# sakehl/SKA-SDP-Accelerate-gridding

Measured on AMD Instinct MI355X. Metric: Mvis/s gridded (w-proj, 4096^2 grid), higher is better.
Workload: dtype f64

## Files before the change

ska-sdp-accelerate-gridding_amd/csrc/tile_sorted.hip:

```cpp
#include "tile_common.h"

namespace gridhip {

__device__ __forceinline__ double readlane_f64(double x, int l)
{
    return __hiloint2double(__builtin_amdgcn_readlane(__double2hiint(x), l),
                            __builtin_amdgcn_readlane(__double2loint(x), l));
}

constexpr int SORTED_IM_OFF = 65528;

__device__ const int cut15[3][16] = {{0, 106, 211, 317, 422, 500, 578, 655, 733, 781, 829, 877, 926, 958, 991, 1024},
                                     {0, 108, 221, 329, 434, 513, 596, 677, 754, 800, 852, 898, 943, 969, 998, 1024},
                                     {0, 100, 202, 303, 401, 480, 562, 641, 718, 769, 824, 875, 925, 957, 992, 1024}};

struct SortedItem {
    int32_t valid, tile, grp, staged;
};

template <int S, bool DEGRID, int ABL = 0, bool AW = false, bool BT = false>
__global__ void __launch_bounds__(1024, 4) tile_grid_sorted_kernel(Geom g, const RecWord *__restrict__ recs,
                                                                const int32_t *__restrict__ bin_start,
                                                                const int32_t *__restrict__ work_start,
                                                                const double2 *__restrict__ gcf,
                                                                double2 *__restrict__ vis,
                                                                double *__restrict__ grid, int nkeys, int batch,
                                                                int32_t *__restrict__ scalars,
                                                                double2 *__restrict__ sorted_vals,
                                                                uint2 *__restrict__ sorted_mo)
{
    extern __shared__ double lds[];
    constexpr int S2 = S * S;
    constexpr int TAIL0 = S2 - ((S2 + 63) / 64 - 1) * 64;
    constexpr int EXTRA = DEGRID ? 0 : (TAIL0 > 32 && TAIL0 <= 34) ? TAIL0 - 32 : (S2 > 256 && TAIL0 <= 2) ? TAIL0 : 0;
    constexpr int S2E = S2 - EXTRA;
    constexpr int NSTEP_ALL = (S2E + 63) / 64;
    constexpr int TAIL = S2E - (NSTEP_ALL - 1) * 64;
    constexpr int MAXST = DEGRID ? 4 : 5;
    constexpr int FP = (NSTEP_ALL + MAXST - 1) / MAXST;
    constexpr int KST = (NSTEP_ALL + FP - 1) / FP;
    constexpr int REM = NSTEP_ALL % FP;
    constexpr int PBASE = NSTEP_ALL / FP;
    constexpr int NSTEP = KST;
    constexpr int LASTS = (REM == 0 ? KST : KST - 1) - 1;
    constexpr bool PAIR = !DEGRID && TAIL == 32;
    const int tid = threadIdx.x, nthr = blockDim.x;
    const int lane = tid & 63, wave = __builtin_amdgcn_readfirstlane(tid >> 6), nw = nthr >> 6;
    const int plane = g.lrows * g.ldw;
    const int IMO = BT ? g.imoff / 8 : SORTED_IM_OFF / 8;
    double *lre = lds, *lim = lds + IMO;
    int32_t *hist = reinterpret_cast<int32_t *>(lim + plane);
    const int hist_words = (nkeys + 1 + 3) & ~3;
    SortedItem *desc = reinterpret_cast<SortedItem *>(hist + hist_words);
    double2 *svals_wg = sorted_vals + (size_t)blockIdx.x * 2 * batch;
    uint2 *smo_wg = sorted_mo + (size_t)blockIdx.x * 2 * batch;
    int32_t *sorig_wg = reinterpret_cast<int32_t *>(sorted_vals) + (size_t)blockIdx.x * 2 * batch;

    constexpr bool STAGE_VALS = !DEGRID && AW;
    constexpr bool STAGE_ORIG = DEGRID && AW;
    const bool solo = nw == 1;
    const bool is_sorter = wave == nw - 1;
    if (is_sorter && !solo && !(g.dbg & 512)) __builtin_amdgcn_s_setprio(3);
    const bool is_walker = solo || !is_sorter;
    const int nwalk = solo ? 1 : nw - 1;
    const int ncell = g.lrows * g.lcols;

    if (blockIdx.x == 0 && tid == 0) {
        long long *st = reinterpret_cast<long long *>(scalars + 20);
        st[0] = (long long)__builtin_amdgcn_s_memtime();
        st[1] = (long long)__builtin_amdgcn_s_memrealtime();
    }
    long long prof[7] = {0, 0, 0, 0, 0, 0, 0}, pt = 0;
#define GH_STAMP(i_)                        \
    if ((ABL & 16) && lane == 0) {          \
        const long long now_ = clock64();   \
        prof[i_] += now_ - pt;              \
        pt = now_;                          \
    }
    if ((ABL & 16) && lane == 0) pt = clock64();

    int32_t *queue = scalars + 4;
    int turn = 0;
    int items_left = ((int)blockIdx.x >= g.npersist) ? g.budget : 0x7fffffff;
    auto prepare = [&](int slot) {
        WorkItem w;
        int grp = 0;
        bool have = false;
        if (items_left <= 0) turn = g.ngroups;
        --items_left;
        while (turn < g.ngroups) {
            grp = (blockIdx.x + turn) % g.ngroups;
            int item = 0;
            if (lane == 0) item = atomicAdd(&queue[grp], 1);
            item = __builtin_amdgcn_readfirstlane(item);
            if (find_work_at(g, bin_start, work_start, grp, item, &w)) {
                have = true;
                break;
            }
            ++turn;
        }
        if (!have) {
            if (lane == 0) desc[slot].valid = 0;
            return;
        }
        GH_STAMP(0)
        const int first_plane = (grp * g.W + g.ngroups - 1) / g.ngroups;
        const int first_slice = first_plane * g.Q * g.Q * g.P;
        double2 *svals = svals_wg + (size_t)slot * batch;
        uint2 *smo = smo_wg + (size_t)slot * batch;
        int32_t *sorig = sorig_wg + (size_t)slot * batch;
        const int b_lo = w.v_lo;
        const int cnt = min(batch, w.v_hi - b_lo);
        for (int i = lane; i <= nkeys; i += 64) hist[i] = 0;
        __builtin_amdgcn_fence(__ATOMIC_ACQ_REL, "wavefront");
        __builtin_amdgcn_wave_barrier();
        for (int r0 = lane; r0 < cnt; r0 += 8 * 64) {
            int key[8];
#pragma unroll
            for (int q = 0; q < 8; ++q) {
                bool off;
                key[q] = load_rec(recs, b_lo + min(r0 + q * 64, cnt - 1), g, &off).kslice - first_slice;
                if (AW) key[q] = (int)((unsigned)key[q] % (unsigned)nkeys);
                if (off) key[q] = -1;
            }
#pragma unroll
            for (int q = 0; q < 8; ++q)
                if (r0 + q * 64 < cnt && (unsigned)key[q] < (unsigned)nkeys) atomicAdd(&hist[key[q]], 1);
        }
        __builtin_amdgcn_fence(__ATOMIC_ACQ_REL, "wavefront");
        __builtin_amdgcn_wave_barrier();
        GH_STAMP(1)
        {
            const int per = (nkeys + 63) / 64;
            const int lo = min(lane * per, nkeys), hi = min(lo + per, nkeys);
            int sum = 0;
            for (int i = lo; i < hi; ++i) sum += hist[i];
            int incl = sum;
#pragma unroll
            for (int off = 1; off < 64; off <<= 1) {
                const int t = __shfl_up(incl, off, 64);
                if (lane >= off) incl += t;
            }
            int base = incl - sum;
            for (int i = lo; i < hi; ++i) {
                const int c = hist[i];
                hist[i] = base;
                base += c;
            }
        }
        __builtin_amdgcn_fence(__ATOMIC_ACQ_REL, "wavefront");
        __builtin_amdgcn_wave_barrier();
        GH_STAMP(2)
        int bad = 0;
        for (int r0 = lane; r0 < cnt; r0 += 8 * 64) {
            VisRec rec[8];
            double2 val[8];
            bool off[8];
#pragma unroll
            for (int q = 0; q < 8; ++q) rec[q] = load_rec(recs, b_lo + min(r0 + q * 64, cnt - 1), g, &off[q]);
            if (STAGE_VALS) {
#pragma unroll
                for (int q = 0; q < 8; ++q) val[q] = (ABL & 8) ? make_double2(1.0, (double)q) : load_nt(vis + rec[q].orig);
            }
#pragma unroll
            for (int q = 0; q < 8; ++q) {
                if (r0 + q * 64 >= cnt) break;
                int key = rec[q].kslice - first_slice;
                if (AW) key = (int)((unsigned)key % (unsigned)nkeys);
                if (off[q] || (unsigned)key >= (unsigned)nkeys) {
                    ++bad;
                    continue;
                }
                const int pos = atomicAdd(&hist[key], 1);
                if ((unsigned)pos < (unsigned)batch) {
                    smo[pos] = make_uint2(((uint32_t)key << 16) | (uint32_t)((rec[q].lxy >> 16) * g.ldw + (rec[q].lxy & 0xffff)),
                                          (uint32_t)(AW ? rec[q].kslice : rec[q].orig));
                    if (STAGE_VALS) svals[pos] = val[q];
                    if (STAGE_ORIG) sorig[pos] = rec[q].orig;
                } else
                    ++bad;
            }
        }
        if (bad) atomicAdd(&scalars[2], bad);
        __builtin_amdgcn_fence(__ATOMIC_ACQ_REL, "wavefront");
        __builtin_amdgcn_wave_barrier();
        if (lane == 0) {
            SortedItem d;
            d.valid = 1;
            d.tile = w.tile;
            d.grp = grp;
            d.staged = hist[nkeys - 1];
            desc[slot] = d;
        }
        GH_STAMP(3)
    };

    int loff[NSTEP];
    const bool tail_ok = lane < TAIL || TAIL == 64;
#pragma unroll
    for (int s = 0; s < NSTEP; ++s) {
        int t = s * 64 + lane;
        if (FP == 1 && s == NSTEP - 1 && !tail_ok) t = PAIR ? s * 64 + lane - 32 : 0;
        loff[s] = (t / S) * g.ldw + (t % S);
    }
    const int ttail = tail_ok ? LASTS * 64 + lane : PAIR ? LASTS * 64 + lane - 32 : 0;
    const int lrow = lane / S, lcol = lane - lrow * S;

    auto walk = [&](int slot, int staged, int first_slice) {
        const double2 *svals = svals_wg + (size_t)slot * batch;
        const uint2 *smo = smo_wg + (size_t)slot * batch;
        const int32_t *sorig = sorig_wg + (size_t)slot * batch;
        int seg_lo, seg_hi;
        if (nwalk == 15 && !DEGRID && !(g.dbg & 256)) {
            seg_lo = (int)(((int64_t)staged * cut15[g.dense][wave]) >> 10);
            seg_hi = (int)(((int64_t)staged * cut15[g.dense][wave + 1]) >> 10);
        } else {
            seg_lo = (int)(((int64_t)staged * wave) / nwalk);
            seg_hi = (int)(((int64_t)staged * (wave + 1)) / nwalk);
        }
        if (seg_lo >= seg_hi) return;
        auto load_list = [&](int b0, uint2 &mo, double2 &v, int32_t &o) {
            const int idx = max(min(b0 + lane, seg_hi - 1), seg_lo);
            mo = smo[idx];
            if (STAGE_VALS) v = svals[idx];
            if (STAGE_ORIG) o = sorig[idx];
        };
        auto load_value = [&](const uint2 &mo, double2 &v) {
            if (!DEGRID && !STAGE_VALS) v = (ABL & 8) ? make_double2(1.0, 2.0) : load_nt(vis + mo.y);
        };
        auto part_step0 = [&](int part) { return FP == 1 ? 0 : part * PBASE + min(part, REM); };
        auto part_nst = [&](int part) { return (FP == 1 || REM == 0 || part < REM) ? KST : KST - 1; };
        auto issue = [&](double2(&k)[NSTEP], int key, int len, int part) {
            key = min(max(key, 0), (AW ? g.nslices : nkeys) - 1);
            asm volatile("" : "+s"(key));
            const double2 *kp = gcf + (size_t)(first_slice + key) * S2 + 64 * part_step0(part);
            if (ABL & 4) {
#pragma unroll
                for (int s = 0; s < NSTEP; ++s) k[s] = make_double2((double)key, (double)(lane + s));
                return;
            }
            const int lofs = len > 0 ? lane : 0, lt = len > 0 ? ttail : 0;
            if (FP == 1) {
#pragma unroll
                for (int s = 0; s < NSTEP - 1; ++s) k[s] = kp[s * 64 + lofs];
                k[NSTEP - 1] = kp[lt];
            } else {
                const bool lastp = part == FP - 1, shortp = part_nst(part) < KST;
#pragma unroll
                for (int s = 0; s < NSTEP; ++s) {
                    int idx = s * 64 + lofs;
                    if (s == LASTS && lastp) idx = lt;
                    if (s == KST - 1 && shortp) idx = 0;
                    k[s] = kp[idx];
                }
            }
        };
        uint2 moN, moNN;
        double2 vN = make_double2(0.0, 0.0), vNN = make_double2(0.0, 0.0);
        int32_t oN = 0, oNN = 0;
        load_list(seg_lo, moN, vN, oN);
        load_list(seg_lo + 64, moNN, vNN, oNN);
        load_value(moN, vN);
        for (int b0 = seg_lo; b0 < seg_hi; b0 += 64) {
            const uint2 mo = moN;
            const double2 vB = vN;
            const int32_t oB = oN;
            moN = moNN;
            vN = vNN;
            oN = oNN;
            load_value(moN, vN);
            load_list(b0 + 128, moNN, vNN, oNN);
            const int bcnt = min(64, seg_hi - b0);
            const uint32_t mykey = AW ? mo.y : mo.x >> 16;
            const uint32_t prevkey = (uint32_t)__shfl_up((int)mykey, 1, 64);
            unsigned long long bits = __ballot(lane < bcnt && (lane == 0 || mykey != prevkey));
            double2 kx[EXTRA > 0 ? EXTRA : 1];
            if (EXTRA > 0) {
                const double2 *kp = gcf + (size_t)(first_slice + min((int)mykey, (AW ? g.nslices : nkeys) - 1)) * S2 + (S2 - EXTRA);
#pragma unroll
                for (int e = 0; e < EXTRA; ++e) kx[e] = (ABL & 4) ? make_double2(1.0, 2.0) : kp[e];
            }
            int lastKey = 0;
            int curKey = 0, curStart = 0, curLen = 0, curPart = FP - 1;
            auto advance = [&](int &key, int &start, int &len, int &part) {
                if (FP > 1 && curLen > 0 && curPart < FP - 1) {
                    ++curPart;
                    key = curKey;
                    start = curStart;
                    len = curLen;
                    part = curPart;
                    return;
                }
                if (bits == 0) {
                    key = lastKey;
                    start = 0;
                    len = 0;
                    if (FP > 1) part = FP - 1;
                    curLen = 0;
                    return;
                }
                start = (int)__builtin_ctzll(bits);
                bits &= bits - 1;
                len = (bits ? (int)__builtin_ctzll(bits) : bcnt) - start;
                key = lastKey = AW ? __builtin_amdgcn_readlane((int)mo.y, start)
                                   : (int)((uint32_t)__builtin_amdgcn_readlane((int)mo.x, start) >> 16);
                if (FP > 1) {
                    part = 0;
                    curKey = key;
                    curStart = start;
                    curLen = len;
                    curPart = 0;
                }
            };
            auto process = [&](const double2(&k)[NSTEP], int start, int len, int part) {
                int lo[NSTEP];
                const bool lastp = FP == 1 || part == FP - 1;
                const bool shortp = FP > 1 && part_nst(part) < KST;
                if (FP == 1) {
#pragma unroll
                    for (int s = 0; s < NSTEP; ++s) lo[s] = loff[s];
                } else {
                    const int st0 = part_step0(part);
#pragma unroll
                    for (int s = 0; s < NSTEP; ++s) {
                        const int tl = 64 * (st0 + s);
                        const int A = tl / S, B = tl - A * S;
                        int lr = lrow, lc = lcol;
                        if (PAIR && s == LASTS && lastp && lane >= 32) {
                            lr = (lane - 32) / S;
                            lc = (lane - 32) - lr * S;
                        }
                        const int carry = (B + lc >= S) ? g.ldw - S : 0;
                        lo[s] = (A + lr) * g.ldw + B + lc + carry;
                    }
                }
                if (!DEGRID) {
                    int i = 0;
                    if (PAIR && lastp) {
                        for (; i + 1 < len; i += 2) {
                            const int j0 = start + i, j1 = j0 + 1;
                            const int lb0 = (int)((uint32_t)__builtin_amdgcn_readlane((int)mo.x, j0) & 0xffff);
                            const int lb1 = (int)((uint32_t)__builtin_amdgcn_readlane((int)mo.x, j1) & 0xffff);
                            const double vx0 = readlane_f64(vB.x, j0), vy0 = readlane_f64(vB.y, j0);
                            const double vx1 = readlane_f64(vB.x, j1), vy1 = readlane_f64(vB.y, j1);
#pragma unroll
                            for (int s = 0; s < LASTS; ++s) {
                                double *cell = lre + (lb0 + lo[s]);
                                if (ABL & 1) continue;
                                __hip_atomic_fetch_add(cell, vx0 * k[s].x - vy0 * k[s].y, __ATOMIC_RELAXED,
                                                       __HIP_MEMORY_SCOPE_WORKGROUP);
                                __hip_atomic_fetch_add(cell + IMO, vx0 * k[s].y + vy0 * k[s].x,
                                                       __ATOMIC_RELAXED, __HIP_MEMORY_SCOPE_WORKGROUP);
                            }
#pragma unroll
                            for (int s = 0; s < LASTS; ++s) {
                                double *cell = lre + (lb1 + lo[s]);
                                if (ABL & 1) continue;
                                __hip_atomic_fetch_add(cell, vx1 * k[s].x - vy1 * k[s].y, __ATOMIC_RELAXED,
                                                       __HIP_MEMORY_SCOPE_WORKGROUP);
                                __hip_atomic_fetch_add(cell + IMO, vx1 * k[s].y + vy1 * k[s].x,
                                                       __ATOMIC_RELAXED, __HIP_MEMORY_SCOPE_WORKGROUP);
                            }
                            const double2 kl = k[LASTS];
                            double re, im;
                            int a;
                            if (lane < 32) {
                                re = vx0 * kl.x - vy0 * kl.y;
                                im = vx0 * kl.y + vy0 * kl.x;
                                a = lb0 + lo[LASTS];
                                asm volatile("" : "+v"(a));
                            } else {
                                re = vx1 * kl.x - vy1 * kl.y;
                                im = vx1 * kl.y + vy1 * kl.x;
                                a = lb1 + lo[LASTS];
                                asm volatile("" : "+v"(a));
                            }
                            if (!(ABL & 1)) {
                                __hip_atomic_fetch_add(lre + a, re, __ATOMIC_RELAXED, __HIP_MEMORY_SCOPE_WORKGROUP);
                                __hip_atomic_fetch_add(lre + a + IMO, im, __ATOMIC_RELAXED,
                                                       __HIP_MEMORY_SCOPE_WORKGROUP);
                            }
                        }
                    }
                    for (; i < len; ++i) {
                        const int j = start + i;
                        const uint32_t m = (uint32_t)__builtin_amdgcn_readlane((int)mo.x, j);
                        const int lbase = (int)(m & 0xffff);
                        const double vx = readlane_f64(vB.x, j), vy = readlane_f64(vB.y, j);
#pragma unroll
                        for (int s = 0; s < NSTEP; ++s) {
                            if (FP > 1 && s == KST - 1 && shortp) continue;
                            const double re = vx * k[s].x - vy * k[s].y;
                            const double im = vx * k[s].y + vy * k[s].x;
                            double *cell = lre + (lbase + lo[s]);
                            if (ABL & 1) {
                                if (re == 1.2345e300 || im == 1.2345e300) *cell = re;
                                continue;
                            }
                            if (TAIL == 64 || s != LASTS || !lastp || tail_ok) {
                                __hip_atomic_fetch_add(cell, re, __ATOMIC_RELAXED, __HIP_MEMORY_SCOPE_WORKGROUP);
                                __hip_atomic_fetch_add(cell + IMO, im, __ATOMIC_RELAXED,
                                                       __HIP_MEMORY_SCOPE_WORKGROUP);
                            }
                        }
                    }
                } else {
                    const double2 kz = tail_ok ? k[LASTS] : make_double2(0.0, 0.0);
                    for (int i = 0; i < len; i += 4) {
                        double sr[4], si[4];
                        int32_t oo[4];
#pragma unroll
                        for (int q = 0; q < 4; ++q) {
                            sr[q] = 0.0;
                            si[q] = 0.0;
                            oo[q] = 0;
                            if (i + q < len) {
                                const int j = start + i + q;
                                const uint32_t m = (uint32_t)__builtin_amdgcn_readlane((int)mo.x, j);
                                const int lbase = (int)(m & 0xffff);
                                oo[q] = __builtin_amdgcn_readlane(STAGE_ORIG ? (int)oB : (int)mo.y, j);
                                double gr[NSTEP], gi[NSTEP];
#pragma unroll
                                for (int s = 0; s < NSTEP; ++s) {
                                    const bool nostep = FP > 1 && s == KST - 1 && shortp;
                                    const bool idle = TAIL != 64 && s == LASTS && lastp && !tail_ok;
                                    const double *cell = lre + (lbase + ((idle || nostep) ? lo[0] : lo[s]));
                                    gr[s] = cell[0];
                                    gi[s] = cell[IMO];
                                }
#pragma unroll
                                for (int s = 0; s < NSTEP; ++s) {
                                    double2 kk = (TAIL != 64 && s == LASTS && lastp) ? kz : k[s];
                                    if (FP > 1 && s == KST - 1 && shortp) kk = make_double2(0.0, 0.0);
                                    sr[q] = fma(kk.x, gr[s], sr[q]);
                                    sr[q] = fma(-kk.y, gi[s], sr[q]);
                                    si[q] = fma(kk.x, gi[s], si[q]);
                                    si[q] = fma(kk.y, gr[s], si[q]);
                                }
                            }
                        }
                        const double rr = wave_sum4_rows(sr[0], sr[1], sr[2], sr[3]);
                        const double ri = wave_sum4_rows(si[0], si[1], si[2], si[3]);
                        const int row = lane >> 4;
                        if ((lane & 15) == 15 && i + row < len) {
                            const int32_t o = row == 0 ? oo[0] : row == 1 ? oo[1] : row == 2 ? oo[2] : oo[3];
                            if (g.P == 1 && FP == 1)
                                __builtin_nontemporal_store(dvec2_t{rr, ri}, reinterpret_cast<dvec2_t *>(vis + o));
                            else {
                                double *dst = reinterpret_cast<double *>(vis + o);
                                unsafeAtomicAdd(dst, rr);
                                unsafeAtomicAdd(dst + 1, ri);
                            }
                        }
                    }
                }
            };

            constexpr int NSETS = 3;
            double2 kS[NSETS][NSTEP];
            int keyS[NSETS], startS[NSETS], lenS[NSETS], partS[NSETS] = {0, 0, 0};
            static_assert(NSETS == 3, "initialiser of partS");
#pragma unroll
            for (int r = 0; r < NSETS - 1; ++r) {
                advance(keyS[r], startS[r], lenS[r], partS[r]);
                issue(kS[r], keyS[r], lenS[r], partS[r]);
            }
            int done = 0;
            for (;;) {
#pragma unroll
                for (int r = 0; r < NSETS; ++r) {
                    const int nx = (r + NSETS - 1) % NSETS;
                    advance(keyS[nx], startS[nx], lenS[nx], partS[nx]);
                    issue(kS[nx], keyS[nx], lenS[nx], partS[nx]);
                    asm volatile("" ::: "memory");
                    __builtin_amdgcn_sched_barrier(0);
                    process(kS[r], startS[r], lenS[r], partS[r]);
                    __builtin_amdgcn_sched_barrier(0);
                    if (FP == 1 || partS[r] == FP - 1) done += lenS[r];
                }
                if (done >= bcnt) break;
            }
            if (done > bcnt) {
#pragma unroll
                for (int r = 0; r < NSETS - 1; ++r) asm volatile("" ::"v"(kS[r][0].x), "v"(kS[r][NSTEP - 1].y));
            }
            if (EXTRA > 0 && !(ABL & 1) && lane < bcnt) {
                const int lb = (int)(mo.x & 0xffff);
#pragma unroll
                for (int e = 0; e < EXTRA; ++e) {
                    const int t = S2 - EXTRA + e;
                    double *cell = lre + (lb + (t / S) * g.ldw + (t % S));
                    __hip_atomic_fetch_add(cell, vB.x * kx[e].x - vB.y * kx[e].y, __ATOMIC_RELAXED,
                                           __HIP_MEMORY_SCOPE_WORKGROUP);
                    __hip_atomic_fetch_add(cell + IMO, vB.x * kx[e].y + vB.y * kx[e].x, __ATOMIC_RELAXED,
                                           __HIP_MEMORY_SCOPE_WORKGROUP);
                }
            }
        }
    };

    const int fl_r0 = (tid >> 1) / g.lcols, fl_c0 = (tid >> 1) - fl_r0 * g.lcols;
    const int fl_dr = (nthr >> 1) / g.lcols, fl_dc = (nthr >> 1) - fl_dr * g.lcols;

    if (is_sorter) prepare(0);
    if (!DEGRID) {
        for (int i = tid; i < plane; i += nthr) {
            lre[i] = 0.0;
            lim[i] = 0.0;
        }
    }
    __syncthreads();
    for (int cur = 0;; cur ^= 1) {
        const SortedItem d = desc[cur];
        if (!d.valid) break;
        const int first_plane = (d.grp * g.W + g.ngroups - 1) / g.ngroups;
        const int first_slice = first_plane * g.Q * g.Q * g.P;
        const int tx = d.tile % g.ntx, ty = d.tile / g.ntx;
        const int64_t ox = (int64_t)tx * g.Tx - g.offx, oy = (int64_t)ty * g.Ty - g.offy;
        if (DEGRID) {
            const double2 *gsrc = reinterpret_cast<const double2 *>(grid);
            for (int c = tid; c < ncell; c += nthr) {
                const int r_ = c / g.lcols, c_ = c - r_ * g.lcols;
                const int64_t gx = ox + c_, gy = oy + r_;
                double2 v = make_double2(0.0, 0.0);
                if (gx >= 0 && gy >= 0 && gx < g.Wd && gy < g.H) v = gsrc[gy * g.Wd + gx];
                lre[r_ * g.ldw + c_] = v.x;
                lim[r_ * g.ldw + c_] = v.y;
            }
            __syncthreads();
        }
        const long long walk_t0 = (ABL & 16) ? clock64() : 0;
        if (is_sorter && !solo) prepare(cur ^ 1);
        if (is_walker) {
            if ((ABL & 16) && wave == 0 && lane == 0) pt = clock64();
            walk(cur, d.staged, first_slice);
            if ((ABL & 16) && wave == 0) GH_STAMP(4)
        }
        if (solo) prepare(cur ^ 1);
        if ((ABL & 16) && lane == 0)
            atomicAdd(reinterpret_cast<unsigned long long *>(scalars + 32) + 8 + wave, (unsigned long long)(clock64() - walk_t0));
        __syncthreads();
        if ((ABL & 16) && wave == 0) GH_STAMP(5)
        if (DEGRID) continue;

        {
            const int comp = tid & 1;
            int r_ = fl_r0, c_ = fl_c0;
            for (int e = tid; e < 2 * ncell; e += nthr) {
                const int64_t gx = ox + c_, gy = oy + r_;
                double *cell = (comp ? lim : lre) + r_ * g.ldw + c_;
                c_ += fl_dc;
                r_ += fl_dr;
                if (c_ >= g.lcols) {
                    c_ -= g.lcols;
                    ++r_;
                }
                const double val = *cell;
                if (val == 0.0) continue;
                *cell = 0.0;
                if ((ABL & 2) || gx < 0 || gy < 0 || gx >= g.Wd || gy >= g.H) continue;
                unsafeAtomicAdd(grid + 2 * (gy * g.Wd + gx) + comp, val);
            }
        }
        __syncthreads();
        if ((ABL & 16) && wave == 0) GH_STAMP(6)
    }
    if (blockIdx.x == 0 && tid == 0) {
        long long *st = reinterpret_cast<long long *>(scalars + 20);
        st[2] = (long long)__builtin_amdgcn_s_memtime();
        st[3] = (long long)__builtin_amdgcn_s_memrealtime();
    }
    if ((ABL & 16) && lane == 0 && (wave == 0 || (is_sorter && !solo))) {
        unsigned long long *out = reinterpret_cast<unsigned long long *>(scalars + 32);
        for (int i = 0; i < 7; ++i)
            if (prof[i]) atomicAdd(&out[i], (unsigned long long)prof[i]);
    }
#undef GH_STAMP
}

bool sorted_plan(const gridhip_ctx *ctx, const Geom &g, int block, int *nkeys, int *batch, size_t *lds_bytes)
{
    if (g.gh != g.gw || g.gh < 5 || g.gh > (g.per_vis ? 16 : 32)) return false;
    const int planes = (g.W + g.ngroups - 1) / g.ngroups + 1;
    const int64_t keys = g.per_vis ? 4096 : (int64_t)planes * g.Q * g.Q * g.P;
    if (keys >= 65536) return false;
    const size_t plane = (size_t)g.lrows * g.ldw * 8;
    if (plane > (size_t)(g.imoff > 0 ? g.imoff : SORTED_IM_OFF)) return false;
    const size_t tile = (size_t)(g.imoff > 0 ? g.imoff : SORTED_IM_OFF) + plane;
    const size_t hist = (size_t)((keys + 1 + 3) & ~3) * 4;
    if (tile + hist + 128 > (size_t)ctx->max_lds) return false;
    (void)block;
    int c = ctx->opt.chunk ? (int)ctx->opt.chunk : 16384;
    c = c < 64 ? 64 : c > 16384 ? 16384 : c;
    *nkeys = (int)keys;
    *batch = c;
    *lds_bytes = tile + hist + 128;
    return true;
}

int launch_tile_grid_sorted(gridhip_ctx *ctx, const Geom &g_in, int block, size_t lds_bytes, int nkeys, int batch,
                            int64_t n, const double *gcf, const double *vis, double *grid, bool degrid)
{
    Geom g = g_in;
    Tables t = tables_of(ctx, g);
    const RecWord *recs = (const RecWord *)ctx->recs.ptr;
    if (g.chunk > batch) return fail(ctx, GRIDHIP_EINVAL, "sorted kernel: chunk %d exceeds its work-item capacity %d", g.chunk, batch);
    if (g.per_vis && g.imoff > 0) return fail(ctx, GRIDHIP_EUNSUPPORTED, "no big-tile form of the aw tile kernel");
    int per_cu = (int)((size_t)ctx->max_lds / lds_bytes);
    per_cu = per_cu < 1 ? 1 : per_cu > 4 ? 4 : per_cu;
    if (per_cu * block > 2048) per_cu = 2048 / block > 0 ? 2048 / block : 1;
    int cus = ctx->num_cu - (int)ctx->opt.reserve_cus;
    if (cus < g.ngroups) cus = g.ngroups;
    int nblk = cus * per_cu;
    nblk = ctx->opt.reserve_cus ? (nblk / g.ngroups) * g.ngroups : ((nblk + g.ngroups - 1) / g.ngroups) * g.ngroups;
    const int most = work_blocks(g, n);
    if (nblk > most) nblk = most > g.ngroups ? (most / g.ngroups) * g.ngroups : g.ngroups;
    g.npersist = nblk;
    g.budget = 0;
    if (ctx->opt.yield_cus > 0 && !ctx->opt.reserve_cus) {
        int k = (((int)ctx->opt.yield_cus + 31) / 32) * 32 * per_cu;
        k = (k / g.ngroups) * g.ngroups;
        if (k > 0 && nblk - k >= g.ngroups) {
            g.npersist = nblk - k;
            g.budget = 8;
            int extra = most - g.npersist;
            extra = extra > 2048 ? 2048 : extra;
            extra = (extra / g.ngroups) * g.ngroups;
            nblk = g.npersist + (extra > k ? extra : k);
        }
    }
    const dim3 gr(nblk), bl(block);
    const size_t nlist = (size_t)nblk * 2 * batch, nvals = g.per_vis ? nlist : 0;
    GH_CHECK(ws_reserve(ctx, ctx->sorted, nvals * 16 + nlist * 8));
    double2 *svals = (double2 *)ctx->sorted.ptr;
    uint2 *smo = (uint2 *)(svals + nvals);
    launch_clear(ctx, t.scalars + 4, 16, (g.dbg & 16) ? t.scalars + 32 : nullptr, (g.dbg & 16) ? 64 : 0);
#define GH_LAUNCH_(S_, D_, B_)                                                                                   \
    do {                                                                                                         \
        GH_CHECK(raise_lds(ctx, tile_grid_sorted_kernel<S_, D_, 0, false, B_>));                                 \
        hipLaunchKernelGGL((tile_grid_sorted_kernel<S_, D_, 0, false, B_>), gr, bl, lds_bytes, ctx->stream, g, recs, \
                           t.bin_start, t.work_start, (const double2 *)gcf, (double2 *)vis, grid, nkeys, batch, \
                           t.scalars, svals, smo);                                                               \
    } while (0)
#define GH_LAUNCH(S_, D_)                \
    do {                                 \
        if (g.imoff > 0)                 \
            GH_LAUNCH_(S_, D_, true);    \
        else                             \
            GH_LAUNCH_(S_, D_, false);   \
    } while (0)
#define GH_LAUNCH_AW_(S_, D_)                                                                                    \
    do {                                                                                                         \
        GH_CHECK(raise_lds(ctx, tile_grid_sorted_kernel<S_, D_, 0, true>));                                      \
        hipLaunchKernelGGL((tile_grid_sorted_kernel<S_, D_, 0, true>), gr, bl, lds_bytes, ctx->stream, g, recs,  \
                           t.bin_start, t.work_start, (const double2 *)gcf, (double2 *)vis, grid, nkeys, batch, \
                           t.scalars, svals, smo);                                                               \
    } while (0)
#define GH_LAUNCH_AW(S_)                 \
    do {                                 \
        if (degrid)                      \
            GH_LAUNCH_AW_(S_, true);     \
        else                             \
            GH_LAUNCH_AW_(S_, false);    \
    } while (0)
#define GH_CASE(S_)             \
    case S_:                    \
        if (g.per_vis)          \
            GH_LAUNCH_AW(S_);   \
        else if (degrid)        \
            GH_LAUNCH(S_, true); \
        else                    \
            GH_LAUNCH(S_, false); \
        break;
#define GH_BIG(S_)                                                                  \
    case S_:                                                                        \
        if (g.per_vis) return fail(ctx, GRIDHIP_EUNSUPPORTED, "aw tile kernel: support %d", g.gh); \
        if (degrid)                                                                 \
            GH_LAUNCH(S_, true);                                                    \
        else                                                                        \
            GH_LAUNCH(S_, false);                                                   \
        break;
#define GH_ABL_BT(A_)                                                                                            \
    if (g.gh == 15 && !degrid && g.imoff > 0 && g.dbg == A_) {                                                   \
        GH_CHECK(raise_lds(ctx, tile_grid_sorted_kernel<15, false, A_, false, true>));                           \
        hipLaunchKernelGGL((tile_grid_sorted_kernel<15, false, A_, false, true>), gr, bl, lds_bytes, ctx->stream, g, recs, \
                           t.bin_start, t.work_start, (const double2 *)gcf, (double2 *)vis, grid, nkeys, batch, \
                           t.scalars, svals, smo);                                                               \
        GH_CHECK_HIP(ctx, hipGetLastError());                                                                    \
        return GRIDHIP_OK;                                                                                       \
    }
#define GH_ABL(A_)                                                                                               \
    if (g.gh == 15 && !degrid && g.imoff == 0 && g.dbg == A_) {                                                  \
        GH_CHECK(raise_lds(ctx, tile_grid_sorted_kernel<15, false, A_>));                                        \
        hipLaunchKernelGGL((tile_grid_sorted_kernel<15, false, A_>), gr, bl, lds_bytes, ctx->stream, g, recs,    \
                           t.bin_start, t.work_start, (const double2 *)gcf, (double2 *)vis, grid, nkeys, batch, \
                           t.scalars, svals, smo);                                                               \
        GH_CHECK_HIP(ctx, hipGetLastError());                                                                    \
        return GRIDHIP_OK;                                                                                       \
    }
#ifdef GRIDHIP_TUNING
    GH_ABL(1) GH_ABL(2) GH_ABL(3) GH_ABL(4) GH_ABL(5) GH_ABL(7) GH_ABL(8) GH_ABL(15) GH_ABL(16) GH_ABL_BT(16)
#endif
#undef GH_ABL
#undef GH_ABL_BT
    switch (g.gh) {
        GH_CASE(5) GH_CASE(6) GH_CASE(7) GH_CASE(8) GH_CASE(9) GH_CASE(10) GH_CASE(11) GH_CASE(12) GH_CASE(13)
        GH_CASE(14) GH_CASE(15) GH_CASE(16)
        GH_BIG(17) GH_BIG(18) GH_BIG(19) GH_BIG(20) GH_BIG(21) GH_BIG(22) GH_BIG(23) GH_BIG(24) GH_BIG(25) GH_BIG(26)
        GH_BIG(27) GH_BIG(28) GH_BIG(29) GH_BIG(30) GH_BIG(31) GH_BIG(32)
        default: return fail(ctx, GRIDHIP_EUNSUPPORTED, "no sorted instantiation for support %d", g.gh);
    }
#undef GH_CASE
#undef GH_BIG
#undef GH_LAUNCH
#undef GH_LAUNCH_
#undef GH_LAUNCH_AW
#undef GH_LAUNCH_AW_
    GH_CHECK_HIP(ctx, hipGetLastError());
    return GRIDHIP_OK;
}

}
```

Before: 9176.

## Pipeline run scheduling across 64-record blocks and carry odd pair tails

```diff
diff --git a/ska-sdp-accelerate-gridding_amd/csrc/tile_sorted.hip b/ska-sdp-accelerate-gridding_amd/csrc/tile_sorted.hip
--- a/ska-sdp-accelerate-gridding_amd/csrc/tile_sorted.hip
+++ b/ska-sdp-accelerate-gridding_amd/csrc/tile_sorted.hip
@@ -6,6 +6,18 @@
 {
     return __hiloint2double(__builtin_amdgcn_readlane(__double2hiint(x), l),
                             __builtin_amdgcn_readlane(__double2loint(x), l));
+}
+
+__device__ __forceinline__ uint32_t reg_move(uint32_t x)
+{
+    uint32_t r;
+    asm("v_mov_b32 %0, %1" : "=v"(r) : "v"(x));
+    return r;
+}
+__device__ __forceinline__ double2 reg_move(const double2 &v)
+{
+    return make_double2(__hiloint2double((int)reg_move((uint32_t)__double2hiint(v.x)), (int)reg_move((uint32_t)__double2loint(v.x))),
+                        __hiloint2double((int)reg_move((uint32_t)__double2hiint(v.y)), (int)reg_move((uint32_t)__double2loint(v.y))));
 }
 
 constexpr int SORTED_IM_OFF = 65528;
@@ -255,34 +267,62 @@
                 }
             }
         };
-        uint2 moN, moNN;
-        double2 vN = make_double2(0.0, 0.0), vNN = make_double2(0.0, 0.0);
-        int32_t oN = 0, oNN = 0;
+        uint2 mo = make_uint2(0, 0), moN, moNN;
+        double2 vB = make_double2(0.0, 0.0), vN = make_double2(0.0, 0.0), vNN = make_double2(0.0, 0.0);
+        int32_t oB = 0, oN = 0, oNN = 0;
+        double2 kx[EXTRA > 0 ? EXTRA : 1];
+        int pb0 = seg_lo - 64, pcnt = 0;
         load_list(seg_lo, moN, vN, oN);
         load_list(seg_lo + 64, moNN, vNN, oNN);
         load_value(moN, vN);
-        for (int b0 = seg_lo; b0 < seg_hi; b0 += 64) {
-            const uint2 mo = moN;
-            const double2 vB = vN;
-            const int32_t oB = oN;
-            moN = moNN;
-            vN = vNN;
-            oN = oNN;
+        auto add_extra = [&]() {
+            if (EXTRA > 0 && !(ABL & 1) && lane < pcnt) {
+                const int lb = (int)(mo.x & 0xffff);
+#pragma unroll
+                for (int e = 0; e < EXTRA; ++e) {
+                    const int t = S2 - EXTRA + e;
+                    double *cell = lre + (lb + (t / S) * g.ldw + (t % S));
+                    __hip_atomic_fetch_add(cell, vB.x * kx[e].x - vB.y * kx[e].y, __ATOMIC_RELAXED,
+                                           __HIP_MEMORY_SCOPE_WORKGROUP);
+                    __hip_atomic_fetch_add(cell + IMO, vB.x * kx[e].y + vB.y * kx[e].x, __ATOMIC_RELAXED,
+                                           __HIP_MEMORY_SCOPE_WORKGROUP);
+                }
+            }
+        };
+        int ahead = 0;
+        unsigned long long gbits = 0;
+        static_assert(!PAIR || FP == 1, "the pair path takes whole runs");
+        bool carry = false;
+        int c_lb = 0;
+        double c_vx = 0.0, c_vy = 0.0;
+        double2 c_k = make_double2(0.0, 0.0);
+        int gb0 = seg_lo - 64, gcnt = 0;
+        auto rotate = [&]() {
+            add_extra();
+            mo = make_uint2(reg_move(moN.x), reg_move(moN.y));
+            vB = reg_move(vN);
+            oB = (int32_t)reg_move((uint32_t)oN);
+            moN = make_uint2(reg_move(moNN.x), reg_move(moNN.y));
+            if (STAGE_VALS) vN = reg_move(vNN);
+            oN = (int32_t)reg_move((uint32_t)oNN);
+            __builtin_amdgcn_sched_barrier(0);
+            pb0 += 64;
+            pcnt = min(64, seg_hi - pb0);
             load_value(moN, vN);
-            load_list(b0 + 128, moNN, vNN, oNN);
-            const int bcnt = min(64, seg_hi - b0);
-            const uint32_t mykey = AW ? mo.y : mo.x >> 16;
-            const uint32_t prevkey = (uint32_t)__shfl_up((int)mykey, 1, 64);
-            unsigned long long bits = __ballot(lane < bcnt && (lane == 0 || mykey != prevkey));
-            double2 kx[EXTRA > 0 ? EXTRA : 1];
+            load_list(pb0 + 128, moNN, vNN, oNN);
             if (EXTRA > 0) {
-                const double2 *kp = gcf + (size_t)(first_slice + min((int)mykey, (AW ? g.nslices : nkeys) - 1)) * S2 + (S2 - EXTRA);
+                const int mykey = (int)(AW ? mo.y : mo.x >> 16);
+                const double2 *kp = gcf + (size_t)(first_slice + min(mykey, (AW ? g.nslices : nkeys) - 1)) * S2 + (S2 - EXTRA);
 #pragma unroll
                 for (int e = 0; e < EXTRA; ++e) kx[e] = (ABL & 4) ? make_double2(1.0, 2.0) : kp[e];
             }
+            ahead = 0;
+        };
+        {
             int lastKey = 0;
             int curKey = 0, curStart = 0, curLen = 0, curPart = FP - 1;
-            auto advance = [&](int &key, int &start, int &len, int &part) {
+            auto advance = [&](int &key, int &start, int &len, int &part, int &newblk, bool first_set) {
+                newblk = 0;
                 if (FP > 1 && curLen > 0 && curPart < FP - 1) {
                     ++curPart;
                     key = curKey;
@@ -291,19 +331,29 @@
                     part = curPart;
                     return;
                 }
-                if (bits == 0) {
-                    key = lastKey;
-                    start = 0;
-                    len = 0;
-                    if (FP > 1) part = FP - 1;
-                    curLen = 0;
-                    return;
-                }
-                start = (int)__builtin_ctzll(bits);
-                bits &= bits - 1;
-                len = (bits ? (int)__builtin_ctzll(bits) : bcnt) - start;
-                key = lastKey = AW ? __builtin_amdgcn_readlane((int)mo.y, start)
-                                   : (int)((uint32_t)__builtin_amdgcn_readlane((int)mo.x, start) >> 16);
+                if (gbits == 0) {
+                    if (!first_set || gb0 + 64 >= seg_hi) {
+                        key = lastKey;
+                        start = 0;
+                        len = 0;
+                        if (FP > 1) part = FP - 1;
+                        curLen = 0;
+                        return;
+                    }
+                    gb0 += 64;
+                    gcnt = min(64, seg_hi - gb0);
+                    newblk = 1;
+                    ahead = 1;
+                    const uint32_t mykey = AW ? moN.y : moN.x >> 16;
+                    const uint32_t prevkey = (uint32_t)__shfl_up((int)mykey, 1, 64);
+                    gbits = __ballot(lane < gcnt && (lane == 0 || mykey != prevkey));
+                }
+                start = (int)__builtin_ctzll(gbits);
+                gbits &= gbits - 1;
+                len = (gbits ? (int)__builtin_ctzll(gbits) : gcnt) - start;
+                const uint32_t gK = ahead ? (AW ? moN.y : moN.x) : (AW ? mo.y : mo.x);
+                key = lastKey = AW ? __builtin_amdgcn_readlane((int)gK, start)
+                                   : (int)((uint32_t)__builtin_amdgcn_readlane((int)gK, start) >> 16);
                 if (FP > 1) {
                     part = 0;
                     curKey = key;
@@ -336,42 +386,30 @@
                 }
                 if (!DEGRID) {
                     int i = 0;
-                    if (PAIR && lastp) {
-                        for (; i + 1 < len; i += 2) {
-                            const int j0 = start + i, j1 = j0 + 1;
-                            const int lb0 = (int)((uint32_t)__builtin_amdgcn_readlane((int)mo.x, j0) & 0xffff);
-                            const int lb1 = (int)((uint32_t)__builtin_amdgcn_readlane((int)mo.x, j1) & 0xffff);
-                            const double vx0 = readlane_f64(vB.x, j0), vy0 = readlane_f64(vB.y, j0);
-                            const double vx1 = readlane_f64(vB.x, j1), vy1 = readlane_f64(vB.y, j1);
+                    if (PAIR) {
+                        auto full_steps = [&](int lb, double vx, double vy) {
 #pragma unroll
                             for (int s = 0; s < LASTS; ++s) {
-                                double *cell = lre + (lb0 + lo[s]);
+                                double *cell = lre + (lb + lo[s]);
                                 if (ABL & 1) continue;
-                                __hip_atomic_fetch_add(cell, vx0 * k[s].x - vy0 * k[s].y, __ATOMIC_RELAXED,
+                                __hip_atomic_fetch_add(cell, vx * k[s].x - vy * k[s].y, __ATOMIC_RELAXED,
                                                        __HIP_MEMORY_SCOPE_WORKGROUP);
-                                __hip_atomic_fetch_add(cell + IMO, vx0 * k[s].y + vy0 * k[s].x,
+                                __hip_atomic_fetch_add(cell + IMO, vx * k[s].y + vy * k[s].x,
                                                        __ATOMIC_RELAXED, __HIP_MEMORY_SCOPE_WORKGROUP);
                             }
-#pragma unroll
-                            for (int s = 0; s < LASTS; ++s) {
-                                double *cell = lre + (lb1 + lo[s]);
-                                if (ABL & 1) continue;
-                                __hip_atomic_fetch_add(cell, vx1 * k[s].x - vy1 * k[s].y, __ATOMIC_RELAXED,
-                                                       __HIP_MEMORY_SCOPE_WORKGROUP);
-                                __hip_atomic_fetch_add(cell + IMO, vx1 * k[s].y + vy1 * k[s].x,
-                                                       __ATOMIC_RELAXED, __HIP_MEMORY_SCOPE_WORKGROUP);
-                            }
-                            const double2 kl = k[LASTS];
+                        };
+                        auto shared_tail = [&](int lb0, double vx0, double vy0, const double2 &k0, int lb1, double vx1,
+                                               double vy1, const double2 &k1) {
                             double re, im;
                             int a;
                             if (lane < 32) {
-                                re = vx0 * kl.x - vy0 * kl.y;
-                                im = vx0 * kl.y + vy0 * kl.x;
+                                re = vx0 * k0.x - vy0 * k0.y;
+                                im = vx0 * k0.y + vy0 * k0.x;
                                 a = lb0 + lo[LASTS];
                                 asm volatile("" : "+v"(a));
                             } else {
-                                re = vx1 * kl.x - vy1 * kl.y;
-                                im = vx1 * kl.y + vy1 * kl.x;
+                                re = vx1 * k1.x - vy1 * k1.y;
+                                im = vx1 * k1.y + vy1 * k1.x;
                                 a = lb1 + lo[LASTS];
                                 asm volatile("" : "+v"(a));
                             }
@@ -380,6 +418,36 @@
                                 __hip_atomic_fetch_add(lre + a + IMO, im, __ATOMIC_RELAXED,
                                                        __HIP_MEMORY_SCOPE_WORKGROUP);
                             }
+                        };
+                        auto rec_of = [&](int j, int &lb, double &vx, double &vy) {
+                            lb = (int)((uint32_t)__builtin_amdgcn_readlane((int)mo.x, j) & 0xffff);
+                            vx = readlane_f64(vB.x, j);
+                            vy = readlane_f64(vB.y, j);
+                        };
+                        if (carry && len > 0) {
+                            int lb1;
+                            double vx1, vy1;
+                            rec_of(start, lb1, vx1, vy1);
+                            full_steps(lb1, vx1, vy1);
+                            shared_tail(c_lb, c_vx, c_vy, c_k, lb1, vx1, vy1, k[LASTS]);
+                            carry = false;
+                            i = 1;
+                        }
+                        for (; i + 1 < len; i += 2) {
+                            int lb0, lb1;
+                            double vx0, vy0, vx1, vy1;
+                            rec_of(start + i, lb0, vx0, vy0);
+                            rec_of(start + i + 1, lb1, vx1, vy1);
+                            full_steps(lb0, vx0, vy0);
+                            full_steps(lb1, vx1, vy1);
+                            shared_tail(lb0, vx0, vy0, k[LASTS], lb1, vx1, vy1, k[LASTS]);
+                        }
+                        if (i < len) {
+                            rec_of(start + i, c_lb, c_vx, c_vy);
+                            full_steps(c_lb, c_vx, c_vy);
+                            c_k = k[LASTS];
+                            carry = true;
+                            i = len;
                         }
                     }
                     for (; i < len; ++i) {
@@ -458,44 +526,42 @@
 
             constexpr int NSETS = 3;
             double2 kS[NSETS][NSTEP];
-            int keyS[NSETS], startS[NSETS], lenS[NSETS], partS[NSETS] = {0, 0, 0};
+            int keyS[NSETS], startS[NSETS], lenS[NSETS], partS[NSETS] = {0, 0, 0}, nbS[NSETS];
             static_assert(NSETS == 3, "initialiser of partS");
 #pragma unroll
             for (int r = 0; r < NSETS - 1; ++r) {
-                advance(keyS[r], startS[r], lenS[r], partS[r]);
+                advance(keyS[r], startS[r], lenS[r], partS[r], nbS[r], r == 0);
                 issue(kS[r], keyS[r], lenS[r], partS[r]);
             }
+            const int total = seg_hi - seg_lo;
             int done = 0;
             for (;;) {
 #pragma unroll
                 for (int r = 0; r < NSETS; ++r) {
                     const int nx = (r + NSETS - 1) % NSETS;
-                    advance(keyS[nx], startS[nx], lenS[nx], partS[nx]);
+                    advance(keyS[nx], startS[nx], lenS[nx], partS[nx], nbS[nx], nx == 0);
                     issue(kS[nx], keyS[nx], lenS[nx], partS[nx]);
                     asm volatile("" ::: "memory");
+                    __builtin_amdgcn_sched_barrier(0);
+                    if (r == 0 && nbS[0]) rotate();
                     __builtin_amdgcn_sched_barrier(0);
                     process(kS[r], startS[r], lenS[r], partS[r]);
                     __builtin_amdgcn_sched_barrier(0);
                     if (FP == 1 || partS[r] == FP - 1) done += lenS[r];
                 }
-                if (done >= bcnt) break;
-            }
-            if (done > bcnt) {
+                if (done >= total) break;
+            }
+            if (done > total) {
 #pragma unroll
                 for (int r = 0; r < NSETS - 1; ++r) asm volatile("" ::"v"(kS[r][0].x), "v"(kS[r][NSTEP - 1].y));
             }
-            if (EXTRA > 0 && !(ABL & 1) && lane < bcnt) {
-                const int lb = (int)(mo.x & 0xffff);
-#pragma unroll
-                for (int e = 0; e < EXTRA; ++e) {
-                    const int t = S2 - EXTRA + e;
-                    double *cell = lre + (lb + (t / S) * g.ldw + (t % S));
-                    __hip_atomic_fetch_add(cell, vB.x * kx[e].x - vB.y * kx[e].y, __ATOMIC_RELAXED,
-                                           __HIP_MEMORY_SCOPE_WORKGROUP);
-                    __hip_atomic_fetch_add(cell + IMO, vB.x * kx[e].y + vB.y * kx[e].x, __ATOMIC_RELAXED,
-                                           __HIP_MEMORY_SCOPE_WORKGROUP);
-                }
-            }
+            if (PAIR && carry && !(ABL & 1) && lane < 32) {
+                double *cell = lre + (c_lb + loff[LASTS]);
+                __hip_atomic_fetch_add(cell, c_vx * c_k.x - c_vy * c_k.y, __ATOMIC_RELAXED, __HIP_MEMORY_SCOPE_WORKGROUP);
+                __hip_atomic_fetch_add(cell + IMO, c_vx * c_k.y + c_vy * c_k.x, __ATOMIC_RELAXED,
+                                       __HIP_MEMORY_SCOPE_WORKGROUP);
+            }
+            add_extra();
         }
     };
 
```

Result: no change. 9230, median of 6 (+0.6%).
